# microsoft/Sora

Hardware: AMD Instinct MI355X
Metric: IQ Msamples/s through 802.11a 54 Mbps RX PHY (higher is better)
Workload: dtype int16 IQ / u8 path metrics

## Files before the change

### sora_amd/csrc/dev_sym11a.h

```cpp
#pragma once
#include "kernels.h"
#include "dev_viterbi.h"
#include "dev_pilot11a.h"

namespace sora {

__device__ __forceinline__ VitJob frame_vitjob(const FrameRow& r)
{
    VitJob J;
    J.valid = 1; J.soft_off = r.slot0 * (uint32_t)kSoftBytesPerSlot; J.nsoft = (uint32_t)r.nsym * 48u * r.nbpsc; J.length = r.length;
    J.dec_off = 0; J.out_off = r.slot0 * (uint32_t)kOutPerSlot; J.code_rate = r.code_rate; J.soft_bits = 3;
    return J;
}

__device__ __forceinline__ unsigned pilot_sgn(unsigned count)
{
    const unsigned w = count < 32 ? kPilotW0 : count < 64 ? kPilotW1 : count < 96 ? kPilotW2 : kPilotW3;
    return (w >> (count & 31u)) & 1u;
}
static __device__ __constant__ PilotPolarity kPilotSgn = kPilotPolarity;
__device__ __forceinline__ int pilot_angle(int th, unsigned count) { return kPilotSgn.neg[count] ? w16(th + 0x8000) : th; }

template <typename COEF> __device__ __forceinline__ pcx sym_freq_comp(uint32_t raw, COEF fq) { return pk_cmul<15>(pk_sra(raw, 1), pk_tw_mul(fq)); }
template <typename COEF> __device__ __forceinline__ pcx sym_equalise(pcx y, COEF ch, int bin)
// ... 18 lines not shown
struct WaveSlots {
    uint32_t first;
    uint32_t my_own;
    unsigned long long owned;
    uint32_t row0;
    bool one_frame;
    __device__ __forceinline__ uint32_t slot(int it, int g) const { return first + 4u * (uint32_t)it + (uint32_t)g; }
    __device__ __forceinline__ uint32_t owner(int it, int g) const { return (uint32_t)__shfl((int)my_own, 4 * it + g); }
    __device__ __forceinline__ unsigned quad(int it) const { return (unsigned)(owned >> (4 * it)) & 0xFu; }
};
__device__ __forceinline__ WaveSlots wave_slots(const RxArgs& A, uint32_t bid)
{
    const int w = threadIdx.x >> 6, lane = threadIdx.x & 63;
    WaveSlots S;
    S.first = (bid * 4u + (uint32_t)w) * (4u * kSlotIters);
    const uint32_t my_slot = S.first + (uint32_t)(lane & 15);
    S.my_own = (lane < 16 && my_slot < A.total_slots) ? A.slot_row[my_slot] : kNoOwner;
    S.owned = __ballot(S.my_own != kNoOwner);
    S.row0 = S.owned ? (uint32_t)__builtin_amdgcn_readlane((int)S.my_own, __builtin_ctzll(S.owned)) : kNoOwner;
    S.one_frame = __ballot(lane < 16 && S.my_own != kNoOwner && S.my_own != S.row0) == 0;
    return S;
}

__device__ __forceinline__ int4 track_advance(int th1, int th2, int th3, int th4, bool act, int& cfo_comp, int& sfo_comp, int& cfo_tr, int& sfo_tr)
{
    const int c0 = cfo_comp, s0 = sfo_comp;
    const int avg = w16((th1 + th2 + th3 + th4) / 4);
    const int del = w16(((th3 - th1) / 28 + (th4 - th2) / 28) >> 1);
    if (act) {
        cfo_tr = w16(cfo_tr + (avg >> 2)); sfo_tr = w16(sfo_tr + (del >> 2));
        cfo_comp = w16(cfo_comp + avg + cfo_tr); sfo_comp = w16(sfo_comp + del + sfo_tr);
    }
    return int4{ c0, s0, act ? avg : 0, act ? del : 0 };
}

__device__ __forceinline__ int4 track_rec4(TrackRec t) { return int4{ t.cfo_comp, t.sfo_comp, t.avg, t.del }; }
__device__ __forceinline__ void sym_back_demap(const Tables& T, const uint8_t* s_demap, const uint32_t v3[3], int4 rec, int nb, int e, uint8_t* dst)
{
    cpx c1[3], c2[3];
#pragma unroll
    for (int m = 0; m < 3; m++) {
        const int bin = carrier_bin48(e + 16 * m);
        const int c = bin < 32 ? bin : bin - 64;
        c1[m] = rot_coeff(T, w16(rec.x + c * rec.y));
        c2[m] = rot_coeff(T, w16(rec.z + c * rec.w));
    }
#pragma unroll
    for (int m = 0; m < 3; m++) {
        const int k = e + 16 * m;
        cpx v = mul_q15(unpack(v3[m]), c1[m]);
        v = mul_q15(v, c2[m]);
        int re = v.re >> 4, im = v.im >> 4;
        re = min(max(re, -128), 127); im = min(max(im, -128), 127);
        const unsigned ur = (unsigned)re & 0xFF, ui = (unsigned)im & 0xFF;
        uint8_t* o = dst + k * nb;
        const int h = nb >> 1;
        o[0] = s_demap[ur];
        if (nb >= 2) {
            o[h] = s_demap[ui];
            if (nb >= 4) {
                const int t1 = nb == 4 ? 256 : 512;
                o[1] = s_demap[t1 + ur]; o[h + 1] = s_demap[t1 + ui];
                if (nb == 6) { o[2] = s_demap[768 + ur]; o[5] = s_demap[768 + ui]; }
            }
        }
    }
}

__device__ __forceinline__ bool deint_packs(int nb, int lane) { return 8 * lane < 48 * nb; }
__device__ __forceinline__ void deint_map_words(const Tables& T, int nb, int lane, uint32_t mp[4])
{
    const uint16_t* map = T.deint + (nb == 1 ? 0 : nb == 2 ? 1 : nb == 4 ? 2 : 3) * 288;
    const bool packs = deint_packs(nb, lane);
#pragma unroll
    for (int t = 0; t < 4; t++) mp[t] = packs ? (uint32_t)map[8 * lane + 2 * t] | ((uint32_t)map[8 * lane + 2 * t + 1] << 16) : 0u;
}
__device__ __forceinline__ uint32_t deint_gather24(const uint8_t* src, const uint32_t mp[4])
{
    uint32_t v[8];
#pragma unroll
    for (int t = 0; t < 4; t++) { v[2 * t] = src[mp[t] & 0xFFFFu]; v[2 * t + 1] = src[mp[t] >> 16]; }
    return soft3_pack8(v);
}

}
```

### sora_amd/csrc/dev_vit16.h

```cpp
#pragma once
#include <hip/hip_runtime.h>
#include "kernels.h"
#include "dev_viterbi.h"

namespace sora {
namespace {

template <int WIN, int LOOK> struct Geom16 {
    static constexpr int kMaxWalk = (WIN + LOOK + 7) / 8 + 2;
    static constexpr int P = kMaxWalk;
    static constexpr int kPathBytes = 40;
};

template <int WIN, int LOOK> struct Lds16 {
    uint16_t ring[Geom16<WIN, LOOK>::P][4][64];
    union {
        uint32_t udump[4][64];
        uint16_t ops[4][24][2];
        uint16_t ops2[2][4][24][2];
    };
    uint32_t path[8][Geom16<WIN, LOOK>::kPathBytes / 4];
};

constexpr unsigned kW[4] = { 0u, 21u, 42u, 63u };

__device__ __forceinline__ unsigned v_of_lane(unsigned l)
{
    const unsigned b0 = l & 1u, b1 = (l >> 1) & 1u, b2 = (l >> 2) & 1u, b3 = (l >> 3) & 1u;
    const unsigned c3 = b2, c1 = b3, c0 = b0 ^ c3, c2 = b1 ^ c3;
    return c0 | (c1 << 1) | (c2 << 2) | (c3 << 3);
}
__device__ __forceinline__ unsigned lane_of_v(unsigned v)
{
    const unsigned c0 = v & 1u, c1 = (v >> 1) & 1u, c2 = (v >> 2) & 1u, c3 = (v >> 3) & 1u;
    return c0 ^ (c2 << 1) ^ (c1 << 3) ^ (c3 ? 7u : 0u);
}
__device__ __forceinline__ unsigned rev6u(unsigned x) { return __brev(x) >> 26; }

template <int CTRL> __device__ __forceinline__ unsigned dppx(unsigned v) { return (unsigned)__builtin_amdgcn_update_dpp(0, (int)v, CTRL, 0xF, 0xF, true); }

__device__ __forceinline__ unsigned partner(unsigned v, int ph)
{
    switch (ph) {
    case 0: return dppx<0x140>(v);
    case 1: return dppx<0x1B>(v);
    case 2: return dppx<0x141>(v);
    case 3: return dppx<0x4E>(v);
    case 4: return dppx<0x128>(v);
    default: return dppx<0xB1>(v);
    }
}

struct Vit16 {
    unsigned U[4];
    unsigned MX[24];
    unsigned MY[6];
    unsigned sadr[3][4];
};

template <int WHICH, int P>
__device__ __forceinline__ void acs16(Vit16& V, int t24, unsigned a, unsigned b, unsigned pos512[3])
{
    const int ph = t24 % 6, k = t24 % 8;
    const unsigned Kp = (WHICH == 0 ? 14u : 7u) * kFld + (kOne << k);
    unsigned bm;
    if (WHICH == 0)      bm = (a ^ V.MX[t24]) + (b ^ V.MY[ph]);
    else if (WHICH == 1) bm = a ^ V.MX[t24];
    else                 bm = b ^ V.MX[t24];
    const unsigned bo = Kp - bm;
    const int rx = ph == 0 ? 2 : ph == 1 ? 1 : 0;
    unsigned N[4];
#pragma unroll
    for (int i = 0; i < 4; i++) {
        const unsigned X = V.U[i], Y = partner(V.U[i ^ rx], ph);
        const bool wb = (kW[i] >> (5 - ph)) & 1u;
        N[i] = wb ? pk_min16(X + bo, Y + bm) : pk_min16(X + bm, Y + bo);
    }
#pragma unroll
    for (int i = 0; i < 4; i++) V.U[i] = N[i];
    if (k == 7) {
        const int jb = t24 / 8;
#pragma unroll
        for (int i = 0; i < 4; i++) {
            const unsigned w = bank_word(V.U[i]);
            const unsigned addr = V.sadr[jb][i] + pos512[jb];
            asm volatile("ds_write_b16 %0, %1" : : "v"(addr), "v"(w) : "memory");
            V.U[i] &= 0xFE00FE00u;
        }
    }
}

__device__ __forceinline__ unsigned row_min_u32(unsigned v)
{
    v = min(v, dppx<0xB1>(v)); v = min(v, dppx<0x4E>(v)); v = min(v, dppx<0x141>(v)); v = min(v, dppx<0x128>(v));
    return v;
}
__device__ __forceinline__ unsigned row_pkmin(unsigned v)
{
    v = pk_min16(v, dppx<0xB1>(v)); v = pk_min16(v, dppx<0x4E>(v)); v = pk_min16(v, dppx<0x141>(v)); v = pk_min16(v, dppx<0x128>(v));
    return v;
}
__device__ __forceinline__ unsigned wave_min_u32(unsigned v) { return (unsigned)__builtin_amdgcn_readfirstlane((int)dpp_min_u32_wave(v)); }
__device__ __forceinline__ unsigned wave_max_u32(unsigned v) { return ~wave_min_u32(~v); }

template <int CR, int WIN, int LOOK, int BITS>
struct Forward16 {
    static constexpr int P = Geom16<WIN, LOOK>::P, GB = Puncture<CR>::GB, GS = Puncture<CR>::GS, CW = Puncture<CR>::CW;
    static constexpr int NV = Puncture<CR>::NV;
    struct Chunk { uint32_t v[CW]; };
    struct Raw { SoftRaw r[NV]; };

    Vit16 V;
    unsigned row, half;
    uint32_t my_j;
    SoftCursor<BITS, CW> cur[NV];
    const uint8_t* soft;
    uint16_t* my_ops;
    const uint4* row_ops;
    uint32_t pos;
    unsigned pos512[3];
    uint32_t tr, nsteps;
    uint32_t next_thr;
    bool all_done;

    __device__ __forceinline__ void init(Lds16<WIN, LOOK>& S, const uint8_t* __restrict__ soft_, uint32_t my_soft_off, uint32_t my_first, uint32_t my_last, unsigned start,
                                         uint32_t nsteps_)
    {
        const unsigned lane = threadIdx.x & 63, l16 = lane & 15;
        row = lane >> 4; half = lane & 1u;
        const unsigned v0 = v_of_lane(l16);
        nsteps = nsteps_;
#pragma unroll
        for (int i = 0; i < 4; i++) V.U[i] = (v0 ^ kW[i]) == 0 ? 0u : start;
        const unsigned ring_base = (unsigned)(uintptr_t)&S.ring[0][0][0];
#pragma unroll
        for (int jb = 0; jb < 3; jb++)
#pragma unroll
            for (int i = 0; i < 4; i++) V.sadr[jb][i] = ring_base + ((row * 64u + rev6u(rol6(v0 ^ kW[i], jb == 0 ? 2 : jb == 1 ? 4 : 0))) << 1);
#pragma unroll
        for (int t = 0; t < 24; t++) {
            const int ph = t % 6, k = t % 8;
            const unsigned n = rol6(v0, ph + 1);
            const bool vb = (v0 >> (5 - ph)) & 1u;
            const unsigned ma = (__popc(n & 0155) & 1) ? 7u * kFld : 0u, mb = (__popc(n & 0117) & 1) ? 7u * kFld : 0u;
            const unsigned mx = Puncture<CR>::which_of(ph) == 2 ? mb : ma;
            V.MX[t] = vb ? ((mx ^ (7u * kFld)) | (kOne << k)) : mx;
            if (t < 6) V.MY[t] = vb ? (mb ^ (7u * kFld)) : mb;
        }
        tr = 0; pos = 0;
        my_j = l16 >> 1;
#pragma unroll
        for (int v = 0; v < NV; v++) cur[v].init(my_soft_off, my_first + my_j + 8u * v, my_last);
        soft = soft_;
        my_ops = &S.ops[row][my_j][half];
        row_ops = reinterpret_cast<const uint4*>(&S.ops[row][0][0]);
        set_row_pos();
    }
    __device__ __forceinline__ bool going() const { return tr < nsteps && !all_done; }

    __device__ __forceinline__ void normalize()
    {
        const unsigned m = row_pkmin(pk_min16(pk_min16(V.U[0], V.U[1]), pk_min16(V.U[2], V.U[3])));
#pragma unroll
        for (int i = 0; i < 4; i++) V.U[i] -= m;
    }
    static __device__ __forceinline__ uint32_t pos_of(uint32_t p, int jb) { const uint32_t q = p + 512u * (uint32_t)jb; return min(q, q - 512u * (uint32_t)P); }
    __device__ __forceinline__ void set_row_pos()
    {
        pos512[0] = pos; pos512[1] = pos_of(pos, 1); pos512[2] = pos_of(pos512[1], 1);
    }
    __device__ __forceinline__ void end_row() { pos = pos_of(pos512[2], 1); set_row_pos(); }
    __device__ __forceinline__ Raw fetch(uint32_t c) const
    {
        Raw R;
#pragma unroll
        for (int v = 0; v < NV; v++) R.r[v] = cur[v].fetch(soft, c);
        return R;
    }
    __device__ __forceinline__ void put(const Raw& R, uint16_t* mine) const
    {
#pragma unroll
        for (int v = 0; v < NV; v++) mine[16 * v] = (uint16_t)cur[v].field(R.r[v]);
    }
    static __device__ __forceinline__ Chunk get(const uint4* table)
    {
        Chunk K;
// ... 142 lines not shown
```

### sora_amd/csrc/dev_viterbi.h

```cpp
#pragma once
#include <hip/hip_runtime.h>
#include "rx_types.h"

namespace sora {

__device__ __forceinline__ uint32_t uni(uint32_t v) { return (uint32_t)__builtin_amdgcn_readfirstlane((int)v); }
__device__ __forceinline__ void lds_fence() { __builtin_amdgcn_fence(__ATOMIC_RELEASE, "wavefront"); __builtin_amdgcn_wave_barrier();
    __builtin_amdgcn_fence(__ATOMIC_ACQUIRE, "wavefront"); }
constexpr uint32_t kNever = 0xFFFFFFFFu;

template <int CR> struct Puncture {
    static constexpr int GB = CR == 0 ? 2 : CR == 2 ? 4 : 3;
    static constexpr int GS = CR == 0 ? 1 : CR == 2 ? 3 : 2;
    static constexpr int CW = 12 / GS * GB;
    static constexpr int NV = (CW + 7) / 8;
    static constexpr int which_of(int ph) { return CR == 0 ? 0 : CR == 1 ? (ph & 1) : ph % 3; }
};

__device__ __forceinline__ unsigned rol6(unsigned v, unsigned r) { r %= 6; return ((v << r) | (v >> (6 - r))) & 63u; }
__device__ __forceinline__ unsigned lane_map(unsigned x) { return x ^ ((x & 4u) ? 3u : 0u); }

__device__ __forceinline__ unsigned dpp_min_u32_wave(unsigned v)
{
    v = min(v, (unsigned)__builtin_amdgcn_update_dpp(0, (int)v, 0xB1, 0xF, 0xF, true));
    v = min(v, (unsigned)__builtin_amdgcn_update_dpp(0, (int)v, 0x4E, 0xF, 0xF, true));
    v = min(v, (unsigned)__builtin_amdgcn_update_dpp(0, (int)v, 0x124, 0xF, 0xF, true));
    v = min(v, (unsigned)__builtin_amdgcn_update_dpp(0, (int)v, 0x128, 0xF, 0xF, true));
    auto r16 = __builtin_amdgcn_permlane16_swap(v, v, false, false);
    v = min(r16[0], r16[1]);
    auto r32 = __builtin_amdgcn_permlane32_swap(v, v, false, false);
    return min(r32[0], r32[1]);
}

typedef unsigned short u16x2_t __attribute__((ext_vector_type(2)));
__device__ __forceinline__ unsigned pk_add16(unsigned a, unsigned b) { return __builtin_bit_cast(unsigned, (u16x2_t)(__builtin_bit_cast(u16x2_t,
        a) + __builtin_bit_cast(u16x2_t, b))); }
__device__ __forceinline__ unsigned pk_sub16(unsigned a, unsigned b) { return __builtin_bit_cast(unsigned, (u16x2_t)(__builtin_bit_cast(u16x2_t,
        a) - __builtin_bit_cast(u16x2_t, b))); }
__device__ __forceinline__ unsigned pk_min16(unsigned a, unsigned b) { return __builtin_bit_cast(unsigned,
        __builtin_elementwise_min(__builtin_bit_cast(u16x2_t, a), __builtin_bit_cast(u16x2_t, b))); }

__device__ __forceinline__ unsigned dpp_pkmin_wave(unsigned v)
{
    v = pk_min16(v, (unsigned)__builtin_amdgcn_update_dpp(0, (int)v, 0xB1, 0xF, 0xF, true));
    v = pk_min16(v, (unsigned)__builtin_amdgcn_update_dpp(0, (int)v, 0x4E, 0xF, 0xF, true));
    v = pk_min16(v, (unsigned)__builtin_amdgcn_update_dpp(0, (int)v, 0x124, 0xF, 0xF, true));
    v = pk_min16(v, (unsigned)__builtin_amdgcn_update_dpp(0, (int)v, 0x128, 0xF, 0xF, true));
    auto r16 = __builtin_amdgcn_permlane16_swap(v, v, false, false);
    v = pk_min16(r16[0], r16[1]);
    auto r32 = __builtin_amdgcn_permlane32_swap(v, v, false, false);
    return pk_min16(r32[0], r32[1]);
}

__device__ __forceinline__ uint32_t soft3_pack8(const uint32_t v[8])
{
    return v[0] | (v[1] << 3) | (v[2] << 6) | (v[3] << 9) | (v[4] << 12) | (v[5] << 15) | (v[6] << 18) | (v[7] << 21);
}
__device__ __forceinline__ void soft3_store8(uint8_t* stream, uint32_t group, uint32_t bits24)
{
    uint8_t* p = stream + 3u * group;
    p[0] = (uint8_t)bits24; p[1] = (uint8_t)(bits24 >> 8); p[2] = (uint8_t)(bits24 >> 16);
}
struct SoftRaw { uint32_t w, sh; };
template <int BITS, int CW> struct SoftCursor {
    static constexpr int ADV = BITS * CW;
    static constexpr bool kConst = ADV % 8 == 0;
    uint32_t off;
    uint32_t pos;
    uint32_t lim;
    uint32_t lsh;
    __device__ __forceinline__ void init(uint32_t stream_off, uint32_t k, uint32_t last)
    {
        const uint32_t t0 = (uint32_t)BITS * min(k, last), tl = (uint32_t)BITS * last;
        if (kConst) { off = stream_off + (t0 >> 3); pos = 0; lim = stream_off + (tl >> 3); lsh = 9u - (t0 & 7u); }
        else { off = stream_off; pos = t0; lim = tl; lsh = 0; }
    }
    __device__ __forceinline__ SoftRaw fetch(const uint8_t* __restrict__ base, uint32_t c) const
    {
        SoftRaw r;
        if (kConst) { r.sh = 0; r.w = *reinterpret_cast<const uint16_t*>(base + min(off + c * (uint32_t)(ADV / 8), lim)); }
        else { const uint32_t t = min(pos + c * (uint32_t)ADV, lim); r.sh = t & 7u; r.w = *reinterpret_cast<const uint16_t*>(base + (off + (t >> 3))); }
        return r;
    }
    __device__ __forceinline__ uint32_t field(const SoftRaw& r) const
    {
        return kConst ? (r.w << lsh) & 0x0E00u : ((r.w >> r.sh) & 7u) << 9;
    }
};

constexpr unsigned kFld = (1u << 9) | (1u << 25);
constexpr unsigned kOne = 0x00020001u;
constexpr unsigned kGuard = 1u << 16;

template <int WIN, int LOOK> struct RingGeom {
    static constexpr int kMaxWalk = (WIN + LOOK + 7) / 8 + 2;
    static constexpr int P = (kMaxWalk + 2) / 3 * 3;
    static constexpr int kEntries = 2 * P * 64;
};

__device__ __forceinline__ unsigned bank_word(unsigned U) { return __builtin_amdgcn_perm(U >> 1, U, 0x0C0C0600u); }

struct VitLane {
    unsigned U;
    unsigned MX[24];
    unsigned MY[6];
    uint16_t* ring;
    unsigned rowpos;
    unsigned sidx[3];
};

template <int WHICH, int P>
__device__ __forceinline__ void acs_step(VitLane& V, int t24, unsigned a, unsigned b)
{
    const int ph = t24 % 6, k = t24 % 8;
    const unsigned Kp = (WHICH == 0 ? 14u : 7u) * kFld + (kOne << k);
    unsigned bm;
    if (WHICH == 0)      bm = (a ^ V.MX[t24]) + (b ^ V.MY[ph]);
    else if (WHICH == 1) bm = a ^ V.MX[t24];
    else                 bm = b ^ V.MX[t24];
    const unsigned bo = Kp - bm;
    unsigned X, Y;
    const int u = (int)V.U;
    switch (ph) {
    case 0: { auto r = __builtin_amdgcn_permlane32_swap(V.U, V.U, false, false); X = r[0]; Y = r[1]; break; }
    case 1: { auto r = __builtin_amdgcn_permlane16_swap(V.U, V.U, false, false); X = r[0]; Y = r[1]; break; }
    case 2: X = V.U; Y = (unsigned)__builtin_amdgcn_update_dpp(0, u, 0x128, 0xF, 0xF, true); break;
    case 3: X = V.U; Y = (unsigned)__builtin_amdgcn_update_dpp(0, u, 0x141, 0xF, 0xF, true); break;
    case 4: X = V.U; Y = (unsigned)__builtin_amdgcn_update_dpp(0, u, 0x4E, 0xF, 0xF, true); break;
    default: X = V.U; Y = (unsigned)__builtin_amdgcn_update_dpp(0, u, 0xB1, 0xF, 0xF, true); break;
    }
    V.U = pk_min16(X + bm, Y + bo);
    if (k == 7) {
        uint16_t* e = V.ring + V.rowpos + (t24 / 8) * 64 + V.sidx[t24 / 8];
        const uint16_t w = (uint16_t)bank_word(V.U);
        e[0] = w; e[P * 64] = w;
        V.U &= 0xFE00FE00u;
    }
}

template <int kMaxWalk>
__device__ __noinline__ void viterbi_trace(unsigned U, const uint16_t* ring, uint32_t tr_, uint32_t ob_, unsigned mA, unsigned mB,
                                           uint32_t cntA_, uint32_t cntB_, uint8_t* outA, uint8_t* outB, uint32_t top_)
{
    const unsigned lane = threadIdx.x & 63;
// ... 212 lines not shown
```

### sora_amd/csrc/dev_vitwin.h

```cpp
#pragma once
#include <hip/hip_runtime.h>
#include <type_traits>
#include "dev_vit16.h"
#include "dev_winplan.h"

namespace sora {

namespace {

struct UnitGeom {
    uint32_t soft_off, last;
    uint32_t i0;
    uint32_t nsteps;
    uint32_t ob;
    uint32_t tr_end;
    uint32_t vstep, estep;
    uint32_t wleft;
    uint32_t vec;
    uint8_t* out;
    uint32_t need;
    uint32_t idx;
    bool valid, first;
};

template <int CR, int WIN, int LOOK>
__device__ __forceinline__ UnitGeom unit_of(const VitJob& J, uint32_t idx, uint32_t uu, uint32_t m, uint32_t nun, uint32_t q, uint32_t vbase, uint8_t* __restrict__ out)
{
    constexpr uint32_t GB = Puncture<CR>::GB, GS = Puncture<CR>::GS;
    UnitGeom g;
    const bool has = uu != kWinNone;
    const uint32_t u = has ? uu : 0u;
    const uint32_t k0 = u * m, k1 = (u + 1u) * m;
    const bool last = u + 1u >= nun;
    const uint32_t b = (uint32_t)WIN * k0 / 24u * 24u;
    const uint32_t s0 = u == 0 ? 0u : b - (uint32_t)kWinWarm;
    g.valid = has; g.first = u == 0;
    g.soft_off = J.soft_off; g.last = max(J.nsoft, 1u) - 1u;
    g.i0 = s0 / GS * GB;
    g.nsteps = has ? J.nsoft / GB * GS - s0 : 0u;
    g.ob = (uint32_t)WIN * k0 - s0;
    g.tr_end = J.length * 8u + 16u + 6u - s0;
    g.vstep = (has && u != 0) ? (uint32_t)kWinWarm : kNever;
    g.estep = (has && !last) ? (uint32_t)WIN * k1 / 24u * 24u - s0 : kNever;
    g.wleft = last ? 0x10000u : m;
    g.vec = vbase + idx * q + u;
    g.out = out + J.out_off + (s0 >> 3);
    g.need = last ? J.nsoft : min(J.nsoft, (((uint32_t)WIN * k1 + (uint32_t)LOOK + 6u + GS) / GS + 1u) * GB);
    g.idx = idx;
    return g;
}

struct UnitRef { uint32_t idx, uu, m, nun; };
template <int CR, int WIN, int LOOK>
__device__ __forceinline__ UnitRef unit_ref(const VitJob& J, uint32_t n, uint32_t p, uint32_t q, bool inside, uint32_t upos, uint32_t idx)
{
    const uint32_t nev = win_events(J.length, CR, WIN, LOOK), m = win_per_unit(nev, q), nun = (nev + m - 1u) / m;
    const uint32_t uu = !inside ? kWinNone : m != 1u ? (upos < nun ? upos : kWinNone) : n == 1u ? win_unit_lone(upos, nun) : (upos < nun ? win_unit_at(upos, nun) : kWinNone);
    return UnitRef{ idx, uu, m, nun };
}
template <int CR, int WIN, int LOOK, typename JOBS>
__device__ __forceinline__ UnitGeom unit_geom(JOBS job_at, uint32_t n, uint32_t p, uint32_t q, uint32_t vbase, uint8_t* __restrict__ out)
{
    const bool inside = p < win_slots(n, q);
    const uint32_t upos = inside ? p / n : 0u, idx = inside ? p - upos * n : 0u;
    const VitJob J = job_at(idx);
    const UnitRef R = unit_ref<CR, WIN, LOOK>(J, n, p, q, inside, upos, idx);
    return unit_of<CR, WIN, LOOK>(J, idx, R.uu, R.m, R.nun, q, vbase, out);
}
template <int CR, int WIN, int LOOK, typename JOBS>
__device__ __forceinline__ UnitGeom unit_geom_direct(JOBS job_at, uint32_t idx, uint32_t u, bool exists, uint32_t q, uint32_t vbase, uint8_t* __restrict__ out)
{
    const VitJob J = job_at(idx);
    const uint32_t nev = win_events(J.length, CR, WIN, LOOK), m = win_per_unit(nev, q), nun = (nev + m - 1u) / m;
    return unit_of<CR, WIN, LOOK>(J, idx, exists && u < nun ? u : kWinNone, m, nun, q, vbase, out);
}

template <int CR, int WIN, int LOOK, int BITS, typename READY>
__device__ __forceinline__ void forward16w(Lds16<WIN, LOOK>& S, const uint8_t* __restrict__ soft, const UnitGeom& GA, const UnitGeom& GB_, uint16_t* __restrict__ vecs, READY ready)
{
    using F16 = Forward16<CR, WIN, LOOK, BITS>;
    using Raw = typename F16::Raw;
    constexpr uint32_t THR = WIN + LOOK + 6;
    const unsigned l16 = threadIdx.x & 15;
    const UnitGeom& Mine = (threadIdx.x & 1u) ? GB_ : GA;
    F16 F;
    F.init(S, soft, Mine.soft_off, Mine.i0, Mine.last, (GA.first ? 0x18u << 9 : 0u) | (GB_.first ? 0x18u << 25 : 0u), wave_max_u32(max(GA.nsteps, GB_.nsteps)));

    uint32_t my_ob = Mine.ob, my_wleft = Mine.wleft;
    const uint32_t my_tr_end = Mine.tr_end;
    bool my_done = !Mine.valid;
    uint32_t vstepA = GA.vstep, vstepB = GB_.vstep, estepA = GA.estep, estepB = GB_.estep;

    auto trace = [&](uint32_t my_cnt, int t24_last) {
        trace16<WIN, LOOK, true>((unsigned)(uintptr_t)&S, F.V.U[0], F.V.U[1], F.V.U[2], F.V.U[3], F.tr, my_ob, F16::pos_of(F.pos, t24_last / 8), (uint32_t)(t24_last % 8), my_cnt,
                                 Mine.out);
    };
    auto next_event = [&]() -> uint32_t {
        uint32_t mine = my_done ? kNever : min(my_ob + THR, my_tr_end);
        mine = min(min(mine, min(vstepA, vstepB)), min(estepA, estepB));
        return wave_min_u32(mine);
    };
    F.next_thr = next_event();
    F.all_done = wave_min_u32(my_done ? 1u : 0u) != 0u;
    auto save = [&](uint32_t vec, int which, bool hi) {
        uint16_t* d = vecs + ((size_t)vec * 2u + (uint32_t)which) * 64u + l16;
#pragma unroll
        for (int i = 0; i < 4; i++) d[16 * i] = (uint16_t)(hi ? F.V.U[i] >> 16 : F.V.U[i]);
    };
    auto check = [&](int t24_last) {
        if (F.tr >= F.next_thr) {
            if (F.tr == vstepA) { save(GA.vec, 0, false); vstepA = kNever; }
            if (F.tr == vstepB) { save(GB_.vec, 0, true); vstepB = kNever; }
            if (F.tr == estepA) { save(GA.vec, 1, false); estepA = kNever; }
            if (F.tr == estepB) { save(GB_.vec, 1, true); estepB = kNever; }
            uint32_t cnt = 0; bool partial = false;
            if (!my_done) {
                if (F.tr >= my_tr_end) { cnt = my_tr_end - my_ob - 6; my_done = true; }
                else if (F.tr >= my_ob + THR) { cnt = WIN; partial = true; }
            }
            if (wave_max_u32(cnt) != 0u) trace(cnt, t24_last);
            if (partial) { my_ob += WIN; if (--my_wleft == 0) my_done = true; }
            F.next_thr = next_event();
            F.all_done = wave_min_u32(my_done ? 1u : 0u) != 0u;
        }
    };

    uint32_t c = 0;
    if (!ready()) return;
    Raw b0 = F.fetch(0), b1 = F.fetch(1), b2, b3;
    while (F.going()) {
        const uint32_t lim = min(F.nsteps, F.next_thr - 1);
        uint32_t rows = lim > F.tr ? (lim - F.tr) / 24 : 0;
        for (; rows > 0; rows--) {
            b2 = F.fetch(c + 2);
            F.fast_chunk(F.unpack(b0), 0);
            b3 = F.fetch(c + 3);
            F.fast_chunk(F.unpack(b1), 1);
            F.end_row();
            b0 = b2; b1 = b3;
            c += 2;
        }
        if (!(F.tr < F.nsteps)) break;
        b2 = F.fetch(c + 2);
        F.chunk(F.unpack(b0), 0, check);
        if (!F.going()) break;
        b3 = F.fetch(c + 3);
        F.chunk(F.unpack(b1), 1, check);
        F.end_row();
        b0 = b2; b1 = b3;
        c += 2;
    }
}

template <int WIN, int LOOK, int BITS, typename JOBSOF, typename READY>
__device__ __forceinline__ void viterbi16w_wave(Lds16<WIN, LOOK>& S, uint32_t wave_index, JOBSOF jobs_of, READY ready, const uint32_t* __restrict__ hdr,
        uint32_t target, uint32_t vstride,
                                                const uint8_t* __restrict__ soft, uint8_t* __restrict__ out, uint16_t* __restrict__ vecs)
{
    const uint32_t n[3] = { hdr[0], hdr[1], hdr[2] };
    const uint32_t q = uni(win_units_per_frame(n[0] + n[1] + n[2], target));
    uint32_t w = uni(wave_index), list = 0;
    while (list < 3 && w >= (win_slots(n[list], q) + 7) / 8) { w -= (win_slots(n[list], q) + 7) / 8; list++; }
    if (list >= 3) return;
    const uint32_t nl = uni(n[list]);
    const auto job_at = jobs_of(list);
    const unsigned lane = threadIdx.x & 63, row = lane >> 4;
    const uint32_t pa = 8u * w + 2u * row, pb = pa + 1u, vbase = list * vstride;
    const uint32_t code_rate = uni(job_at(0).code_rate);
    auto run = [&](auto cr) {
        constexpr int CR = decltype(cr)::value;
        UnitGeom A = unit_geom<CR, WIN, LOOK>(job_at, nl, pa, q, vbase, out), B = unit_geom<CR, WIN, LOOK>(job_at, nl, pb, q, vbase, out);
        if (__ballot(A.valid || B.valid) == 0) return;
        if (!B.valid) { const bool v = false; B = A; B.valid = v; B.vstep = B.estep = kNever; B.nsteps = 0; }
        if (!A.valid) { const bool v = false; const UnitGeom T = B; A = T; A.valid = v; A.vstep = A.estep = kNever; A.nsteps = 0; }
        forward16w<CR, WIN, LOOK, BITS>(S, soft, A, B, vecs, [&]() { return ready(A, B, list); });
    };
    if (code_rate == 0) run(std::integral_constant<int, 0>{});
    else if (code_rate == 1) run(std::integral_constant<int, 1>{});
    else run(std::integral_constant<int, 2>{});
}

template <int WIN, int LOOK, int BITS>
__device__ __forceinline__ void viterbi16w_body(const VitJob* __restrict__ jobs, const uint32_t* __restrict__ hdr, uint32_t jstride, uint32_t target, uint32_t vstride,
                                                const uint8_t* __restrict__ soft, uint8_t* __restrict__ out, uint16_t* __restrict__ vecs)
{
    __shared__ Lds16<WIN, LOOK> S;
    auto jobs_of = [&](uint32_t list) { const VitJob* __restrict__ jl = jobs + (size_t)list * jstride; return [jl](uint32_t idx) { return jl[idx]; }; };
    auto ready = [](const UnitGeom&, const UnitGeom&, uint32_t) { return true; };
    viterbi16w_wave<WIN, LOOK, BITS>(S, blockIdx.x, jobs_of, ready, hdr, target, vstride, soft, out, vecs);
}

}

}
```

### sora_amd/csrc/k_rx.hip

```cpp
#include <hip/hip_runtime.h>
#include <utility>
#include "kernels.h"
#include "dev_sym11a.h"
#include "dev_viterbi.h"
#include "dev_winplan.h"
#include "dev_vitwin.h"

namespace sora {

struct FrameLds {
    uint32_t eq[4][4][64];
    uint8_t  soft[4][4][288];
    uint8_t  demap[1024];
    int4     trk[4][4];
    int      nsym_of[4];
    short    st0[4][4];
};
template <bool SHARED>
__device__ __forceinline__ void frame_symbols(const RxArgs& A, uint32_t j, FrameLds& lds, bool valid = true)
{
    uint32_t (&s_eq)[4][4][64] = lds.eq; uint8_t (&s_soft)[4][4][288] = lds.soft; const uint8_t* s_demap = lds.demap;
    const int w = threadIdx.x >> 6, lane = threadIdx.x & 63, g = lane >> 4, e = lane & 15;
    const Tables& T = A.T;
    const uint32_t f = valid ? A.joblist[j] : 0u;
    FrameRow r = A.frames[f];
    if (!valid) { r.nsym = 0; r.nbpsc = 1; }
    if (lane == 0 && valid) A.jobs[j] = frame_vitjob(r);
    const FrameCtx* fx = A.fctx + f;
    const uint32_t* iq = A.iq + A.caps[r.capture].offset;
    const Fft64TwPk W = fft64_twiddles_pk(T, e);
    PkTw fq[4], ch[4];
#pragma unroll
    for (int m = 0; m < 4; m++) { fq[m] = pk_tw_mul(fx->freq[e + 16 * m]); ch[m] = pk_tw_mul(fx->chan[e + 16 * m]); }
    const int nb = __builtin_amdgcn_readfirstlane((int)r.nbpsc), ncbps = 48 * nb, nsym = __builtin_amdgcn_readfirstlane((int)r.nsym);
    uint32_t mp[4];
    const bool packs = deint_packs(nb, lane);
    deint_map_words(T, nb, lane, mp);
    uint8_t* dst = A.soft + (size_t)r.slot0 * kSoftBytesPerSlot;
    const int pk = lane & 3;
    const int pbin = pk == 0 ? 43 : pk == 1 ? 57 : pk == 2 ? 7 : 21, pc = pk == 0 ? -21 : pk == 1 ? -7 : pk == 2 ? 7 : 21;
    int cfo_comp = r.cfo_comp, sfo_comp = r.sfo_comp, cfo_tr = r.cfo_tracker, sfo_tr = r.sfo_tracker;
    unsigned symbol_count = 0;

    const uint32_t str_shift = A.str >> 1;
    auto load_samples = [&](int s0, uint32_t raw[4]) {
        const uint32_t p0 = r.data_start + __umul24(80u, (uint32_t)min(s0 + g, nsym)) + 8u + (uint32_t)e;
#pragma unroll
        for (int m = 0; m < 4; m++) raw[m] = iq[(p0 + 16u * (uint32_t)m) << str_shift];
    };
    int nsym_loop = nsym, nsym_f = nsym;
    if (SHARED) {
        if (lane == 0) { lds.nsym_of[w] = nsym; lds.st0[w][0] = (short)cfo_comp; lds.st0[w][1] = (short)sfo_comp; lds.st0[w][2] = (short)cfo_tr; lds.st0[w][3] = (short)sfo_tr; }
        __syncthreads();
        nsym_loop = max(max(lds.nsym_of[0], lds.nsym_of[1]), max(lds.nsym_of[2], lds.nsym_of[3]));
        const int fr = (lane >> 2) & 3;
        nsym_f = lds.nsym_of[fr];
        cfo_comp = lds.st0[fr][0]; sfo_comp = lds.st0[fr][1]; cfo_tr = lds.st0[fr][2]; sfo_tr = lds.st0[fr][3];
    }
    uint32_t raw[4] = { 0u, 0u, 0u, 0u };
    if (1 <= nsym) load_samples(1, raw);
    for (int s0 = 1; s0 <= nsym_loop; s0 += 4) {
        const int sym = s0 + g;
        const bool active = sym <= nsym;
        const bool mine = s0 <= nsym;
        int4 rec = { 0, 0, 0, 0 };
        if (mine) {
            pcx x[4], Y[4];
#pragma unroll
            for (int m = 0; m < 4; m++) x[m] = sym_freq_comp(raw[m], fq[m]);
            if (s0 + 4 <= nsym) load_samples(s0 + 4, raw);
            fft64_core_pk(x, s_eq[w][g], e, W, wave_lds_sync);
#pragma unroll
            for (int q = 0; q < 4; q++) Y[q] = s_eq[w][g][__brev((unsigned)(e + 16 * q)) >> 26];
            wave_lds_sync();
#pragma unroll
            for (int q = 0; q < 4; q++) s_eq[w][g][e + 16 * q] = sym_equalise(Y[q], ch[q], e + 16 * q);
            wave_lds_sync();
        }
        if (SHARED) {
            __syncthreads();
            if (w == 0) {
                const int fr = (lane >> 2) & 3;
#pragma unroll
                for (int gg = 0; gg < 4; gg++) {
                    const cpx p = mul_q15(unpack(s_eq[fr][gg][pbin]), rot_coeff(T, w16(cfo_comp + pc * sfo_comp)));
                    const int th = pilot_angle(pk == 3 ? uatan2(T, -p.im, -p.re) : uatan2(T, p.im, p.re), (symbol_count + (unsigned)gg) % 127u);
                    int th1 = __builtin_amdgcn_update_dpp(0, th, 0x00, 0xF, 0xF, true), th2 = __builtin_amdgcn_update_dpp(0, th, 0x55, 0xF, 0xF, true);
                    int th3 = __builtin_amdgcn_update_dpp(0, th, 0xAA, 0xF, 0xF, true), th4 = __builtin_amdgcn_update_dpp(0, th, 0xFF, 0xF, 0xF, true);
                    asm volatile("" : "+v"(th1), "+v"(th2), "+v"(th3), "+v"(th4));
                    const int4 t = track_advance(th1, th2, th3, th4, s0 + gg <= nsym_f, cfo_comp, sfo_comp, cfo_tr, sfo_tr);
                    if (lane < 16 && pk == 0) lds.trk[fr][gg] = t;
                }
            }
            symbol_count = (symbol_count + 4u) % 127u;
            __syncthreads();
            rec = lds.trk[w][g];
        } else {
            int4 t[4];
#pragma unroll
            for (int gg = 0; gg < 4; gg++) {
                t[gg] = int4{ cfo_comp, sfo_comp, 0, 0 };
                if (s0 + gg <= nsym) {
                    const cpx p = mul_q15(unpack(s_eq[w][gg][pbin]), rot_coeff(T, w16(cfo_comp + pc * sfo_comp)));
                    const int th = pilot_angle(pk == 3 ? uatan2(T, -p.im, -p.re) : uatan2(T, p.im, p.re), symbol_count);
                    symbol_count++; if (symbol_count >= 127) symbol_count = 0;
                    t[gg] = track_advance(__builtin_amdgcn_readlane(th, 0), __builtin_amdgcn_readlane(th, 1), __builtin_amdgcn_readlane(th, 2), __builtin_amdgcn_readlane(th, 3),
                                          true, cfo_comp, sfo_comp, cfo_tr, sfo_tr);
                }
            }
            rec = t[0];
            if (g == 1) rec = t[1]; else if (g == 2) rec = t[2]; else if (g == 3) rec = t[3];
        }
        if (!mine) continue;
        if (active) {
            uint32_t v3[3];
#pragma unroll
            for (int m = 0; m < 3; m++) v3[m] = s_eq[w][g][carrier_bin48(e + 16 * m)];
            sym_back_demap(T, s_demap, v3, rec, nb, e, s_soft[w][g]);
        }
        wave_lds_sync();
        {
            const int nact = min(4, nsym - s0 + 1);
            const uint32_t sym_bytes = 3u * (uint32_t)ncbps / 8u;
            uint8_t* d = dst + (size_t)(s0 - 1) * sym_bytes;
            for (int gs = 0; gs < nact; gs++, d += sym_bytes)
                if (packs) soft3_store8(d, (uint32_t)lane, deint_gather24(s_soft[w][gs], mp));
        }
        wave_lds_sync();
    }
}
__global__ void __launch_bounds__(256) k_frame(RxArgs A)
{
    __shared__ FrameLds lds;
    reinterpret_cast<uint32_t*>(lds.demap)[threadIdx.x] = reinterpret_cast<const uint32_t*>(A.T.demap)[threadIdx.x];
    __syncthreads();
    if (!locate_job(blockIdx.x * 4, A.njobs).ok) return;
    const JobRef jr = locate_job(blockIdx.x * 4 + (threadIdx.x >> 6), A.njobs);
    frame_symbols<true>(A, jr.ok ? jr.list * A.nrows + jr.idx : 0u, lds, jr.ok);
}

typedef uint32_t u32x4_t __attribute__((ext_vector_type(4)));
__device__ __forceinline__ void store16_through(uint4* p, uint4 v)
{
    const u32x4_t x = { v.x, v.y, v.z, v.w };
    asm volatile("global_store_dwordx4 %0, %1, off sc1\n\ts_nop 1" : : "v"(p), "v"(x) : "memory");
}
__device__ __forceinline__ void store4_through(uint32_t* p, uint32_t v) { __hip_atomic_store(p, v, __ATOMIC_RELAXED, __HIP_MEMORY_SCOPE_AGENT); }

template <bool THROUGH>
__device__ __forceinline__ void sym_front_block(const RxArgs& A, uint32_t bid, uint32_t (*s_eq)[4][64])
{
    const int w = threadIdx.x >> 6, lane = threadIdx.x & 63, g = lane >> 4, e = lane & 15;
    const Tables& T = A.T;
    const WaveSlots S = wave_slots(A, bid);
    if (S.owned == 0) return;
    uint32_t own[kSlotIters];
#pragma unroll
    for (int it = 0; it < kSlotIters; it++) own[it] = S.owner(it, g);
    const Fft64TwPk W = fft64_twiddles_pk(T, e);
    uint32_t* sl = s_eq[w][g];
    uint4* eq4 = reinterpret_cast<uint4*>(A.eq);
    auto store = [&](uint32_t slot, const uint32_t o[4]) {
        if (THROUGH) store16_through(eq4 + ((size_t)slot * 16u + (uint32_t)e), uint4{ o[0], o[1], o[2], o[3] });
        else eq4[(size_t)slot * 16u + (uint32_t)e] = uint4{ o[0], o[1], o[2], o[3] };
        auto pilot = [&](uint32_t k, uint32_t v) { if (THROUGH) store4_through(A.pil + ((size_t)slot * 4u + k), v); else A.pil[(size_t)slot * 4u + k] = v; };
        if (e == 10) pilot(0u, o[3]);
        if (e == 14) pilot(1u, o[1]);
        if (e == 1)  pilot(2u, o[3]);
        if (e == 5)  pilot(3u, o[1]);
    };
    if (S.one_frame) {
        const FrameRow& r = A.frames[S.row0];
        const uint32_t* iq = A.iq + A.caps[r.capture].offset;
        const uint32_t ds = r.data_start, s0 = r.slot0, str = A.str;
        const FrameCtx* fx = A.fctx + S.row0;
        uint32_t raw[kSlotIters][4];
#pragma unroll
        for (int it = 0; it < kSlotIters; it++) {
            const uint32_t p0 = ds + 80u * (S.slot(it, g) - s0) + 8u;
#pragma unroll
            for (int m = 0; m < 4; m++) raw[it][m] = own[it] != kNoOwner ? iq[(size_t)(p0 + (uint32_t)(e + 16 * m)) * str] : 0u;
        }
        PkTw fq[4], ch[4];
#pragma unroll
        for (int m = 0; m < 4; m++) { fq[m] = pk_tw_mul(fx->freq[e + 16 * m]); ch[m] = pk_tw_mul(fx->chan[4 * e + m]); }
#pragma unroll
        for (int it = 0; it < kSlotIters; it++) {
            if (S.quad(it) == 0) continue;
            uint32_t o[4];
            sym_front_quad(raw[it], fq, ch, sl, e, W, o);
            if (own[it] != kNoOwner) store(S.slot(it, g), o);
        }
        return;
    }
#pragma unroll 1
    for (int it = 0; it < kSlotIters; it++) {
        if (S.quad(it) == 0) continue;
        const uint32_t ow = S.owner(it, g);
        const bool mine = ow != kNoOwner;
        const uint32_t slot = S.slot(it, g);
        uint32_t raw[4] = { 0u, 0u, 0u, 0u };
        PkTw fq[4], ch[4];
        const FrameCtx* fx = A.fctx + (mine ? ow : 0u);
        if (mine) {
            const FrameRow& r = A.frames[ow];
            const uint32_t* iq = A.iq + A.caps[r.capture].offset;
            const uint32_t p0 = r.data_start + 80u * (slot - r.slot0) + 8u;
#pragma unroll
            for (int m = 0; m < 4; m++) raw[m] = iq[(size_t)(p0 + (uint32_t)(e + 16 * m)) * A.str];
// ... 752 lines not shown
```

### sora_amd/csrc/k_vit16.hip

```cpp
#include <hip/hip_runtime.h>

#include "dev_vit16.h"

namespace sora {

namespace {

template <int CR, int WIN, int LOOK, int BITS>
__device__ __forceinline__ void forward16(Lds16<WIN, LOOK>& S, const uint8_t* __restrict__ soft, uint32_t my_soft_off, uint32_t my_nsoft,
                                          uint32_t nstepsA, uint32_t nstepsB, uint32_t my_tr_end, bool my_valid, uint8_t* my_out)
{
    using F16 = Forward16<CR, WIN, LOOK, BITS>;
    using Chunk = typename F16::Chunk;
    using Raw = typename F16::Raw;
    constexpr int GS = F16::GS;
    F16 F;
    F.init(S, soft, my_soft_off, 0, max(my_nsoft, 1u) - 1u, 0x18u * kFld, wave_max_u32(max(nstepsA, nstepsB)));

    uint32_t ob = 0;
    bool my_done = !my_valid;

    auto trace = [&](uint32_t my_cnt, int t24_last) {
        trace16<WIN, LOOK>((unsigned)(uintptr_t)&S, F.V.U[0], F.V.U[1], F.V.U[2], F.V.U[3], F.tr, ob, F16::pos_of(F.pos, t24_last / 8), (uint32_t)(t24_last % 8), my_cnt, my_out);
    };
    auto next_event = [&]() -> uint32_t {
        const uint32_t mine = my_done ? kNever : my_tr_end;
        return min(ob + (uint32_t)(WIN + LOOK + 6), wave_min_u32(mine));
    };
    F.next_thr = next_event();
    F.all_done = wave_min_u32(my_done ? 1u : 0u) != 0u;
    auto check = [&](int t24_last) {
        if (F.tr >= F.next_thr) {
            const bool partial = F.tr >= ob + (uint32_t)(WIN + LOOK + 6);
            uint32_t cnt = 0;
            if (!my_done) {
                if (F.tr >= my_tr_end) { cnt = my_tr_end - ob - 6; my_done = true; }
                else if (partial) cnt = WIN;
            }
            if (wave_max_u32(cnt) != 0u) trace(cnt, t24_last);
            if (partial) ob += WIN;
            F.next_thr = next_event();
            F.all_done = wave_min_u32(my_done ? 1u : 0u) != 0u;
        }
    };

    uint16_t* my_ops2[2] = { &S.ops2[0][F.row][F.my_j][F.half], &S.ops2[1][F.row][F.my_j][F.half] };
    const uint4* row_ops2[2] = { reinterpret_cast<const uint4*>(&S.ops2[0][F.row][0][0]), reinterpret_cast<const uint4*>(&S.ops2[1][F.row][0][0]) };
    auto stage = [&](const Raw& R, int t) { F.put(R, my_ops2[t]); };
    auto collect = [&](int t) -> Chunk { lds_fence(); return F16::get(row_ops2[t]); };
    auto fast_chunk_mid = [&](const Chunk& K, int h, Chunk& Knext, int tnext) {
#pragma unroll
        for (int g = 0; g < 12 / GS; g++) {
            if (g == (12 / GS) / 2) Knext = collect(tnext);
            F.group(K, h, g * GS);
        }
        F.tr += 12;
    };

    uint32_t c = 0;
    Raw b0 = F.fetch(0), b1 = F.fetch(1), b2, b3;
    while (F.going()) {
        const uint32_t lim = min(F.nsteps, F.next_thr - 1);
        uint32_t rows = lim > F.tr ? (lim - F.tr) / 24 : 0;
        if (rows >= 2) {
            Chunk Ka, Kb;
            b2 = F.fetch(c + 2);
            stage(b0, 0); Ka = collect(0); lds_fence();
            for (; rows >= 2; rows -= 2) {
                b3 = F.fetch(c + 3); stage(b1, 1); fast_chunk_mid(Ka, 0, Kb, 1);
                b0 = F.fetch(c + 4); stage(b2, 0); fast_chunk_mid(Kb, 1, Ka, 0);
                F.end_row();
                b1 = F.fetch(c + 5); stage(b3, 1); fast_chunk_mid(Ka, 0, Kb, 1);
                b2 = F.fetch(c + 6); stage(b0, 0); fast_chunk_mid(Kb, 1, Ka, 0);
                F.end_row();
                c += 4;
            }
            lds_fence();
        }
        if (!(F.tr < F.nsteps)) break;
        b2 = F.fetch(c + 2);
        if (rows) F.fast_chunk(F.unpack(b0), 0); else F.chunk(F.unpack(b0), 0, check);
        if (!F.going()) break;
        b3 = F.fetch(c + 3);
        if (rows) F.fast_chunk(F.unpack(b1), 1); else F.chunk(F.unpack(b1), 1, check);
        F.end_row();
        b0 = b2; b1 = b3;
        c += 2;
    }
}

template <int WIN, int LOOK, int BITS>
__device__ __forceinline__ void viterbi16_body(const VitJob* __restrict__ jobs, const uint32_t* __restrict__ njobs3, uint32_t njobs_single, uint32_t stride,
                                               const uint8_t* __restrict__ soft, uint8_t* __restrict__ out)
{
    __shared__ Lds16<WIN, LOOK> S;
    uint32_t n[3] = { njobs_single, 0, 0 };
    if (njobs3) { n[0] = njobs3[0]; n[1] = njobs3[1]; n[2] = njobs3[2]; }
    uint32_t w = uni(blockIdx.x), list = 0;
    while (list < 3 && w >= (n[list] + 7) / 8) { w -= (n[list] + 7) / 8; list++; }
    if (list >= 3) return;
    const uint32_t njobs = uni(n[list]);
    jobs += (size_t)list * stride;
    const unsigned lane = threadIdx.x & 63, row = lane >> 4, half = lane & 1u;
    const uint32_t fa = 8u * w + 2u * row, fb = fa + 1u;
    const bool hasA = fa < njobs, hasB = fb < njobs;
    const VitJob& GA = jobs[hasA ? fa : 8u * w];
    const VitJob& GBj = jobs[hasB ? fb : (hasA ? fa : 8u * w)];
    const uint32_t code_rate = uni(jobs[8u * w].code_rate);
    const uint32_t gsd = code_rate == 0 ? 2u : code_rate == 2 ? 4u : 3u, gss = code_rate == 0 ? 1u : code_rate == 2 ? 3u : 2u;
    const uint32_t nstepsA = hasA ? GA.nsoft / gsd * gss : 0u, nstepsB = hasB ? GBj.nsoft / gsd * gss : 0u;
    const VitJob& Mine = half ? GBj : GA;
    const bool my_valid = half ? hasB : hasA;
    const uint32_t my_tr_end = Mine.length * 8u + 16u + 6u;
    uint8_t* my_out = out + Mine.out_off;
    if (code_rate == 0)      forward16<0, WIN, LOOK, BITS>(S, soft, Mine.soft_off, Mine.nsoft, nstepsA, nstepsB, my_tr_end, my_valid, my_out);
    else if (code_rate == 1) forward16<1, WIN, LOOK, BITS>(S, soft, Mine.soft_off, Mine.nsoft, nstepsA, nstepsB, my_tr_end, my_valid, my_out);
    else                     forward16<2, WIN, LOOK, BITS>(S, soft, Mine.soft_off, Mine.nsoft, nstepsA, nstepsB, my_tr_end, my_valid, my_out);
}

}

__global__ void __launch_bounds__(64) k_viterbi16(const VitJob* __restrict__ jobs, const uint32_t* __restrict__ njobs3, uint32_t njobs_single, uint32_t stride,
        const uint8_t* __restrict__ soft, uint8_t* __restrict__ out)
{ viterbi16_body<256, 24, 3>(jobs, njobs3, njobs_single, stride, soft, out); }
__global__ void __launch_bounds__(64) k_viterbi16_11n(const VitJob* __restrict__ jobs, const uint32_t* __restrict__ njobs3, uint32_t njobs_single,
// ... 5 lines not shown
```

Baseline: 54160.

## Batch deinterleave LDS gathers and replace wave reductions with ballots

The frame symbol kernel now precomputes LDS byte addresses for the deinterleave map. For full four-symbol groups it issues the gathers two symbols at a time and waits once before packing and storing, so LDS latency overlaps instead of being paid per symbol. In the Viterbi kernels, the all-done and trace-needed checks use a ballot instead of a DPP wave min/max reduction. The earliest frame end is also cached and recomputed only when some lane finishes. Explicit sched_barrier and waitcnt constrain compiler scheduling, which could hurt if it interferes with other overlap.

```diff
diff --git a/sora_amd/csrc/dev_sym11a.h b/sora_amd/csrc/dev_sym11a.h
--- a/sora_amd/csrc/dev_sym11a.h
+++ b/sora_amd/csrc/dev_sym11a.h
@@ -124,5 +124,29 @@
     for (int t = 0; t < 4; t++) { v[2 * t] = src[mp[t] & 0xFFFFu]; v[2 * t + 1] = src[mp[t] >> 16]; }
     return soft3_pack8(v);
 }
+typedef __attribute__((address_space(3))) const uint8_t lds_cu8;
+__device__ __forceinline__ void deint_map_addrs(const Tables& T, int nb, int lane, const uint8_t* sym0, uint32_t ad[8])
+{
+    uint32_t mp[4];
+    deint_map_words(T, nb, lane, mp);
+    const uint32_t base = (uint32_t)(uintptr_t)sym0;
+#pragma unroll
+    for (int t = 0; t < 4; t++) { ad[2 * t] = base + (mp[t] & 0xFFFFu); ad[2 * t + 1] = base + (mp[t] >> 16); }
+}
+__device__ __forceinline__ void deint_read8_at(const uint32_t ad[8], uint32_t off, uint32_t v[8])
+{
+#pragma unroll
+    for (int t = 0; t < 8; t++) v[t] = ((lds_cu8*)(uintptr_t)ad[t])[off];
+}
+__device__ __forceinline__ uint32_t deint_gather24_at(const uint32_t ad[8], uint32_t off)
+{
+    uint32_t v[8];
+    deint_read8_at(ad, off, v);
+    return soft3_pack8(v);
+}
+__device__ __forceinline__ void lds_reads_landed()
+{
+    __builtin_amdgcn_sched_barrier(0); __builtin_amdgcn_s_waitcnt(0xC07F); __builtin_amdgcn_sched_barrier(0);
+}
 
 }
diff --git a/sora_amd/csrc/dev_vit16.h b/sora_amd/csrc/dev_vit16.h
--- a/sora_amd/csrc/dev_vit16.h
+++ b/sora_amd/csrc/dev_vit16.h
@@ -102,6 +102,7 @@
 }
 __device__ __forceinline__ unsigned wave_min_u32(unsigned v) { return (unsigned)__builtin_amdgcn_readfirstlane((int)dpp_min_u32_wave(v)); }
 __device__ __forceinline__ unsigned wave_max_u32(unsigned v) { return ~wave_min_u32(~v); }
+__device__ __forceinline__ uint32_t earliest_end16(bool done, uint32_t tr_end) { return wave_min_u32(done ? kNever : tr_end); }
 
 template <int CR, int WIN, int LOOK, int BITS>
 struct Forward16 {
diff --git a/sora_amd/csrc/dev_viterbi.h b/sora_amd/csrc/dev_viterbi.h
--- a/sora_amd/csrc/dev_viterbi.h
+++ b/sora_amd/csrc/dev_viterbi.h
@@ -60,6 +60,11 @@
 {
     uint8_t* p = stream + 3u * group;
     p[0] = (uint8_t)bits24; p[1] = (uint8_t)(bits24 >> 8); p[2] = (uint8_t)(bits24 >> 16);
+}
+__device__ __forceinline__ void soft3_store8_at(uint8_t* p, uint32_t bits24)
+{
+    const uint16_t lo = (uint16_t)bits24;
+    __builtin_memcpy(p, &lo, 2); p[2] = (uint8_t)(bits24 >> 16);
 }
 struct SoftRaw { uint32_t w, sh; };
 template <int BITS, int CW> struct SoftCursor {
diff --git a/sora_amd/csrc/dev_vitwin.h b/sora_amd/csrc/dev_vitwin.h
--- a/sora_amd/csrc/dev_vitwin.h
+++ b/sora_amd/csrc/dev_vitwin.h
@@ -101,7 +101,7 @@
         return wave_min_u32(mine);
     };
     F.next_thr = next_event();
-    F.all_done = wave_min_u32(my_done ? 1u : 0u) != 0u;
+    F.all_done = __ballot(!my_done) == 0;
     auto save = [&](uint32_t vec, int which, bool hi) {
         uint16_t* d = vecs + ((size_t)vec * 2u + (uint32_t)which) * 64u + l16;
 #pragma unroll
@@ -118,10 +118,10 @@
                 if (F.tr >= my_tr_end) { cnt = my_tr_end - my_ob - 6; my_done = true; }
                 else if (F.tr >= my_ob + THR) { cnt = WIN; partial = true; }
             }
-            if (wave_max_u32(cnt) != 0u) trace(cnt, t24_last);
+            if (__ballot(cnt != 0u) != 0) trace(cnt, t24_last);
             if (partial) { my_ob += WIN; if (--my_wleft == 0) my_done = true; }
             F.next_thr = next_event();
-            F.all_done = wave_min_u32(my_done ? 1u : 0u) != 0u;
+            F.all_done = __ballot(!my_done) == 0;
         }
     };
 
diff --git a/sora_amd/csrc/k_rx.hip b/sora_amd/csrc/k_rx.hip
--- a/sora_amd/csrc/k_rx.hip
+++ b/sora_amd/csrc/k_rx.hip
@@ -16,6 +16,7 @@
     int      nsym_of[4];
     short    st0[4][4];
 };
+constexpr int kDeintGroup = 2;
 template <bool SHARED>
 __device__ __forceinline__ void frame_symbols(const RxArgs& A, uint32_t j, FrameLds& lds, bool valid = true)
 {
@@ -33,10 +34,11 @@
 #pragma unroll
     for (int m = 0; m < 4; m++) { fq[m] = pk_tw_mul(fx->freq[e + 16 * m]); ch[m] = pk_tw_mul(fx->chan[e + 16 * m]); }
     const int nb = __builtin_amdgcn_readfirstlane((int)r.nbpsc), ncbps = 48 * nb, nsym = __builtin_amdgcn_readfirstlane((int)r.nsym);
-    uint32_t mp[4];
+    uint32_t ad[8];
     const bool packs = deint_packs(nb, lane);
-    deint_map_words(T, nb, lane, mp);
-    uint8_t* dst = A.soft + (size_t)r.slot0 * kSoftBytesPerSlot;
+    deint_map_addrs(T, nb, lane, s_soft[w][0], ad);
+    uint8_t* dst = A.soft + (size_t)(uint32_t)__builtin_amdgcn_readfirstlane((int)r.slot0) * kSoftBytesPerSlot;
+    const uint32_t lane3 = 3u * (uint32_t)lane;
     const int pk = lane & 3;
     const int pbin = pk == 0 ? 43 : pk == 1 ? 57 : pk == 2 ? 7 : 21, pc = pk == 0 ? -21 : pk == 1 ? -7 : pk == 2 ? 7 : 21;
     int cfo_comp = r.cfo_comp, sfo_comp = r.sfo_comp, cfo_tr = r.cfo_tracker, sfo_tr = r.sfo_tracker;
@@ -123,8 +125,23 @@
             const int nact = min(4, nsym - s0 + 1);
             const uint32_t sym_bytes = 3u * (uint32_t)ncbps / 8u;
             uint8_t* d = dst + (size_t)(s0 - 1) * sym_bytes;
-            for (int gs = 0; gs < nact; gs++, d += sym_bytes)
-                if (packs) soft3_store8(d, (uint32_t)lane, deint_gather24(s_soft[w][gs], mp));
+            if (nact == 4) {
+                if (packs) {
+#pragma unroll
+                    for (int h = 0; h < 4; h += kDeintGroup) {
+                        uint32_t v[kDeintGroup][8];
+#pragma unroll
+                        for (int gs = 0; gs < kDeintGroup; gs++) deint_read8_at(ad, 288u * (uint32_t)(h + gs), v[gs]);
+                        lds_reads_landed();
+#pragma unroll
+                        for (int gs = 0; gs < kDeintGroup; gs++) soft3_store8_at(d + (lane3 + (uint32_t)(h + gs) * sym_bytes), soft3_pack8(v[gs]));
+                        if (h + kDeintGroup < 4) __builtin_amdgcn_sched_barrier(0);
+                    }
+                }
+            } else {
+                for (int gs = 0; gs < nact; gs++)
+                    if (packs) soft3_store8_at(d + (lane3 + (uint32_t)gs * sym_bytes), deint_gather24_at(ad, 288u * (uint32_t)gs));
+            }
         }
         wave_lds_sync();
     }
diff --git a/sora_amd/csrc/k_vit16.hip b/sora_amd/csrc/k_vit16.hip
--- a/sora_amd/csrc/k_vit16.hip
+++ b/sora_amd/csrc/k_vit16.hip
@@ -23,24 +23,23 @@
     auto trace = [&](uint32_t my_cnt, int t24_last) {
         trace16<WIN, LOOK>((unsigned)(uintptr_t)&S, F.V.U[0], F.V.U[1], F.V.U[2], F.V.U[3], F.tr, ob, F16::pos_of(F.pos, t24_last / 8), (uint32_t)(t24_last % 8), my_cnt, my_out);
     };
-    auto next_event = [&]() -> uint32_t {
-        const uint32_t mine = my_done ? kNever : my_tr_end;
-        return min(ob + (uint32_t)(WIN + LOOK + 6), wave_min_u32(mine));
-    };
+    uint32_t first_end = earliest_end16(my_done, my_tr_end);
+    auto next_event = [&]() -> uint32_t { return min(ob + (uint32_t)(WIN + LOOK + 6), first_end); };
     F.next_thr = next_event();
-    F.all_done = wave_min_u32(my_done ? 1u : 0u) != 0u;
+    F.all_done = __ballot(!my_done) == 0;
     auto check = [&](int t24_last) {
         if (F.tr >= F.next_thr) {
             const bool partial = F.tr >= ob + (uint32_t)(WIN + LOOK + 6);
             uint32_t cnt = 0;
+            bool ended = false;
             if (!my_done) {
-                if (F.tr >= my_tr_end) { cnt = my_tr_end - ob - 6; my_done = true; }
+                if (F.tr >= my_tr_end) { cnt = my_tr_end - ob - 6; my_done = ended = true; }
                 else if (partial) cnt = WIN;
             }
-            if (wave_max_u32(cnt) != 0u) trace(cnt, t24_last);
+            if (__ballot(cnt != 0u) != 0) trace(cnt, t24_last);
             if (partial) ob += WIN;
+            if (__ballot(ended) != 0) { first_end = earliest_end16(my_done, my_tr_end); F.all_done = __ballot(!my_done) == 0; }
             F.next_thr = next_event();
-            F.all_done = wave_min_u32(my_done ? 1u : 0u) != 0u;
         }
     };
 
```

After: 54530, median of 2. No clear change (+0.7%).
